# imdea-software/legosnark

Measured on AMD Instinct MI355X. Metric: alt_bn128 G1 MSM point-scalar pairs/s at n=2^20, higher is better.
Workload: dtype u32 limbs (254-bit Montgomery integers)

## Files before the change

### legosnark_amd/csrc/msm.hip

```cpp
#include <hip/hip_runtime.h>
#include <stdint.h>
#include <stdio.h>
#include <stdlib.h>
#include <string.h>
#include <algorithm>
#include <type_traits>
#include <vector>

#include "curves.h"
#include "fp29x2l.h"
#include "fs29.h"
#include "glv.h"
#include "msm.h"
#include "msm_plan.h"

namespace lsa {


template <class F, int K>
__global__ __launch_bounds__(256) void k_normalize(const Jac<F> *__restrict__ in, Aff<F> *__restrict__ out, size_t n) {
    size_t t = (size_t)blockIdx.x * blockDim.x + threadIdx.x;
    size_t base = t * K;
    if (base >= n) return;
    F prod[K];
// ... 447 lines not shown
            uint32_t gex = gi - gv, lex = li - lv;
            for (unsigned w = 0; w < wv; w++) { gex += wtot[0][w]; lex += wtot[1][w]; }
            lstart[threadIdx.x] = lex;
            lcur[threadIdx.x] = lex;
            gdst[threadIdx.x] = gex + tile_base[(size_t)t * pitch + threadIdx.x];
            if (blockIdx.x == 0) offs_c[threadIdx.x] = gex;
            if (threadIdx.x == Bc - 1) lstart[Bc] = lex + lv;
        }
    }
    __syncthreads();
    const size_t lo = (size_t)t * PART_TILE;
    const uint32_t fine_bits = cm.sh_hi;
    const uint32_t tlow = t & ((1u << (16 - fine_bits)) - 1);
    for (uint32_t j = 0; j < PART_TILE / 1024; j++) {
        const uint32_t il = threadIdx.x + j * 1024;
        const size_t i = lo + il;
        if (i >= n) break;
        const uint32_t seg = segment_of(segs, (uint32_t)i);
        wide_digits(scalars[i], pl, seg * B, [&](unsigned k, int32_t sd) {
            if (sd != 0) {
                const uint32_t b = (uint32_t)(sd < 0 ? -sd : sd) - 1;
                const uint32_t pos = atomicAdd(&lcur[cm.bin(b)], 1u);
                stage[pos] = (tlow << (16 + fine_bits)) | (cm.fine(b) << 16) | (k << 12) | (sd < 0 ? 0x800u : 0u) | il;
            }
        });
    }
    __syncthreads();
    for (uint32_t sg = threadIdx.x >> 5; sg < Bc; sg += 32) {
        const uint32_t a = lstart[sg], e = lstart[sg + 1], g = gdst[sg];
        for (uint32_t x = a + (lane & 31); x < e; x += 32) recs[g + (x - a)] = stage[x];
    }
}

__global__ __launch_bounds__(1024) void k_fine_sort_part(const uint32_t *__restrict__ recs, const uint32_t *__restrict__ offs_c,
                                                         const uint32_t *__restrict__ hist_c, const uint32_t *__restrict__ tile_base,
                                                         uint32_t pitch, uint32_t T, CoarseMap cm, SegList segs, uint32_t win_stride, uint32_t stage_cap,
                                                         uint32_t *__restrict__ entries, uint32_t *__restrict__ hist, uint32_t *__restrict__ offs) {
    __builtin_amdgcn_s_setprio(3);
    extern __shared__ __attribute__((aligned(16))) uint32_t sm[];
    __shared__ uint32_t wsum[16];
    const uint32_t sg = blockIdx.x, lo = offs_c[sg], ns = hist_c[sg];
    const uint32_t fine_bits = cm.sh_hi, FM = 1u << fine_bits, fmask = FM - 1, tbits = 16 - fine_bits;
    const uint32_t F = 1u << cm.bits(sg), bucket0 = cm.first(sg);
    uint32_t *cnt = sm, *cur = sm + FM, *col = sm + 2 * FM, *stage = col + T + 1;
    const unsigned lane = threadIdx.x & 63, wv = threadIdx.x >> 6;
    for (uint32_t x = threadIdx.x; x < F; x += 1024) cnt[x] = 0;
    for (uint32_t x = threadIdx.x; x < T; x += 1024) col[x] = tile_base[(size_t)x * pitch + sg];
    if (threadIdx.x == 0) col[T] = ns;
    auto scan_counters = [&]() {
        const uint32_t per = (F + 1023) >> 10, f0 = threadIdx.x * per;
        uint32_t sum = 0;
        for (uint32_t q = 0; q < per; q++) if (f0 + q < F) sum += cnt[f0 + q];
        uint32_t incl = sum;
#pragma unroll
        for (int d = 1; d < 64; d <<= 1) {
            const uint32_t u = __shfl_up(incl, d, 64);
            if ((int)lane >= d) incl += u;
        }
        if (lane == 63) wsum[wv] = incl;
        __syncthreads();
        uint32_t run = incl - sum;
        for (unsigned w = 0; w < wv; w++) run += wsum[w];
        for (uint32_t q = 0; q < per; q++) {
            if (f0 + q >= F) break;
            const uint32_t c = cnt[f0 + q];
            cur[f0 + q] = run;
            hist[(size_t)bucket0 + f0 + q] = c;
            offs[(size_t)bucket0 + f0 + q] = lo + run;
            run += c;
        }
    };
    auto entry_of = [&](uint32_t r, uint32_t p2) {
        uint32_t a = 0, e = (T + (1u << tbits) - 1) >> tbits;
        while (e - a > 1) {
            const uint32_t m = (a + e) >> 1;
            if (col[m << tbits] <= p2) a = m; else e = m;
        }
        const uint32_t i = ((a << tbits) | (r >> (16 + fine_bits))) * PART_TILE + (r & 0x7ffu);
        const uint32_t local = i - segs.off[segment_of(segs, i)];
        return (local + ((r >> 12) & 15u) * win_stride) | ((r & 0x800u) << 20);
    };
    if (ns <= stage_cap) {
        constexpr uint32_t NR = PART_STAGE / 1024;
        uint32_t r[NR];
#pragma unroll
        for (uint32_t u = 0; u < NR; u++) { const uint32_t p2 = threadIdx.x + u * 1024; r[u] = p2 < ns ? recs[lo + p2] : 0u; }
        __syncthreads();
        uint16_t rk[NR];
#pragma unroll
        for (uint32_t u = 0; u < NR; u++) {
            rk[u] = 0;
            if (threadIdx.x + u * 1024 < ns) rk[u] = (uint16_t)atomicAdd(&cnt[(r[u] >> 16) & fmask], 1u);
        }
        __syncthreads();
        scan_counters();
        __syncthreads();
#pragma unroll
        for (uint32_t u = 0; u < NR; u++) {
            const uint32_t p2 = threadIdx.x + u * 1024;
            if (p2 < ns) stage[cur[(r[u] >> 16) & fmask] + rk[u]] = entry_of(r[u], p2);
        }
        __syncthreads();
        for (uint32_t x = threadIdx.x; x < ns; x += 1024) entries[lo + x] = stage[x];
        return;
    }
    __syncthreads();
    constexpr uint32_t UNR = 8;
    for (uint32_t p0 = threadIdx.x; p0 < ns; p0 += 1024 * UNR) {
        uint32_t r[UNR];
#pragma unroll
        for (uint32_t u = 0; u < UNR; u++) { const uint32_t p2 = p0 + u * 1024; r[u] = p2 < ns ? recs[lo + p2] : 0u; }
#pragma unroll
        for (uint32_t u = 0; u < UNR; u++) if (p0 + u * 1024 < ns) (void)lds_inc_rank(cnt, (r[u] >> 16) & fmask);
    }
    __syncthreads();
    scan_counters();
    __syncthreads();
    for (uint32_t p0 = threadIdx.x; p0 < ns; p0 += 1024 * UNR) {
        uint32_t r[UNR];
#pragma unroll
        for (uint32_t u = 0; u < UNR; u++) { const uint32_t p2 = p0 + u * 1024; r[u] = p2 < ns ? recs[lo + p2] : 0u; }
#pragma unroll
        for (uint32_t u = 0; u < UNR; u++) {
            const uint32_t p2 = p0 + u * 1024;
            if (p2 >= ns) break;
            entries[lo + lds_inc_rank(cur, (r[u] >> 16) & fmask)] = entry_of(r[u], p2);
        }
    }
}

template <class Rec>
struct RecOps;
template <>
struct RecOps<uint64_t> {
    static constexpr uint32_t NF = 128;
    static __device__ __forceinline__ uint32_t fine(uint64_t r) { return (uint32_t)(r >> 32); }
    static __device__ __forceinline__ uint32_t entry(uint64_t r) { return (uint32_t)r; }
};
template <>
struct RecOps<uint32_t> {
    static constexpr uint32_t NF = 64;
    static __device__ __forceinline__ uint32_t fine(uint32_t r) { return (r >> 25) & 63u; }
    static __device__ __forceinline__ uint32_t entry(uint32_t r) { return r & 0x81ffffffu; }
};
template <class Rec>
__global__ __launch_bounds__(1024) void k_fine_sort(const Rec *__restrict__ recs, const uint32_t *__restrict__ offs_c,
                                                    const uint32_t *__restrict__ hist_c, uint32_t *__restrict__ entries,
                                                    uint32_t *__restrict__ hist, uint32_t *__restrict__ offs) {
    using O = RecOps<Rec>;
    constexpr uint32_t NF = O::NF;
// ... 1 lines not shown
    const uint32_t bin = blockIdx.x, lo = offs_c[bin], n = hist_c[bin];
    if (threadIdx.x < NF) cnt[threadIdx.x] = 0;
    __syncthreads();
    for (uint32_t j = threadIdx.x; j < n; j += 1024) atomicAdd(&cnt[O::fine(recs[lo + j])], 1u);
    __syncthreads();
    if (threadIdx.x < 64) {
        constexpr uint32_t PER = NF / 64;
        uint32_t c[PER], tot = 0;
#pragma unroll
        for (uint32_t q = 0; q < PER; q++) { c[q] = cnt[PER * threadIdx.x + q]; tot += c[q]; }
        uint32_t incl = tot;
#pragma unroll
        for (int d = 1; d < 64; d <<= 1) {
            uint32_t t = __shfl_up(incl, d, 64);
            if ((int)threadIdx.x >= d) incl += t;
        }
        uint32_t ex = incl - tot;
#pragma unroll
        for (uint32_t q = 0; q < PER; q++) {
            cur[PER * threadIdx.x + q] = ex;
            hist[(size_t)bin * NF + PER * threadIdx.x + q] = c[q];
            offs[(size_t)bin * NF + PER * threadIdx.x + q] = lo + ex;
            ex += c[q];
        }
    }
    __syncthreads();
    for (uint32_t j = threadIdx.x; j < n; j += 1024) {
        const Rec r = recs[lo + j];
        const uint32_t pos = atomicAdd(&cur[O::fine(r)], 1u);
        entries[lo + pos] = O::entry(r);
    }
}

__device__ __forceinline__ uint32_t size_bin(uint32_t cnt, uint32_t bin_shift) { return ((cnt - 1) >> bin_shift) + 1; }
template <class C>
__global__ __launch_bounds__(256) void k_size_hist(const uint32_t *__restrict__ hist, uint32_t nb, uint32_t thr, uint32_t *__restrict__ bin_count,
                                                   uint32_t group_size, uint32_t bin_shift) {
    bin_count += (group_size ? (blockIdx.x * 2048u) / group_size : 0u) * SIZE_BINS;
    __shared__ uint32_t lcnt[SIZE_BINS];
    for (uint32_t t = threadIdx.x; t < SIZE_BINS; t += 256) lcnt[t] = 0;
    __syncthreads();
    const uint32_t base = blockIdx.x * 2048 + threadIdx.x;
#pragma unroll
    for (int j = 0; j < 8; j++) {
        uint32_t g = base + j * 256;
        if (g < nb) { uint32_t cnt = hist[g]; if (cnt > 0 && cnt <= thr) atomicAdd(&lcnt[size_bin(cnt, bin_shift)], 1u); }
    }
    __syncthreads();
    for (uint32_t t = threadIdx.x; t < SIZE_BINS; t += 256) if (lcnt[t]) atomicAdd(&bin_count[t], lcnt[t]);
}
__global__ __launch_bounds__(256) void k_size_scan(const uint32_t *__restrict__ bin_count, uint32_t *__restrict__ bin_start, uint32_t ngroups) {
    __shared__ uint32_t lds[4];
    uint32_t carry = 0;
    for (uint32_t gidx = 0; gidx < ngroups; gidx++) {
        const uint32_t *bc = bin_count + gidx * SIZE_BINS;
        uint32_t *bs = bin_start + gidx * SIZE_BINS;
        uint32_t v[4], s = 0;
#pragma unroll
        for (int j = 0; j < 4; j++) {
            int bin = (int)SIZE_BINS - 1 - (int)(threadIdx.x * 4 + j);
            v[j] = (bin >= 1) ? bc[bin] : 0;
            s += v[j];
        }
        uint32_t tot;
        uint32_t run = carry + block_exclusive_scan_256(s, lds, &tot);
#pragma unroll
        for (int j = 0; j < 4; j++) {
            int bin = (int)SIZE_BINS - 1 - (int)(threadIdx.x * 4 + j);
            if (bin >= 1) bs[bin] = run;
            run += v[j];
        }
        carry += tot;
    }
    if (threadIdx.x == 0) bin_start[0] = carry;
}
template <class C>
__global__ __launch_bounds__(256) void k_size_scatter(const uint32_t *__restrict__ hist, uint32_t nb, uint32_t thr, const uint32_t *__restrict__ bin_start,
                                                      uint32_t *__restrict__ bin_cursor, uint32_t *__restrict__ perm,
                                                      uint32_t *__restrict__ heavy_list, uint32_t *__restrict__ heavy_count,
                                                      typename C::Acc *__restrict__ buckets, uint32_t group_size, uint32_t bin_shift,
                                                      uint32_t split) {
    const uint32_t goff = (group_size ? (blockIdx.x * 2048u) / group_size : 0u) * SIZE_BINS;
    bin_start += goff;
    bin_cursor += goff;
    __shared__ uint32_t lcnt[SIZE_BINS];
    for (uint32_t t = threadIdx.x; t < SIZE_BINS; t += 256) lcnt[t] = 0;
    __syncthreads();
    const uint32_t base = blockIdx.x * 2048 + threadIdx.x;
    uint32_t cnt[8], rank[8];
#pragma unroll
    for (int j = 0; j < 8; j++) {
        uint32_t g = base + j * 256;
        cnt[j] = 0; rank[j] = 0;
        if (g < nb) {
            cnt[j] = hist[g];
            if (cnt[j] == 0) { for (uint32_t h = 0; h < split; h++) buckets[(size_t)g * split + h] = C::inf(); }
            else if (cnt[j] > thr) heavy_list[atomicAdd(heavy_count, 1u)] = g;
            else rank[j] = atomicAdd(&lcnt[size_bin(cnt[j], bin_shift)], 1u);
        }
    }
    __syncthreads();
    for (uint32_t t = threadIdx.x; t < SIZE_BINS; t += 256) {
        uint32_t c = lcnt[t];
        lcnt[t] = c ? atomicAdd(&bin_cursor[t], c) : 0;
    }
    __syncthreads();
#pragma unroll
    for (int j = 0; j < 8; j++) {
        uint32_t g = base + j * 256;
        if (g < nb && cnt[j] > 0 && cnt[j] <= thr) {
            const uint32_t bin = size_bin(cnt[j], bin_shift);
            perm[bin_start[bin] + lcnt[bin] + rank[j]] = g;
        }
    }
}

typedef uint32_t u32x4 __attribute__((ext_vector_type(4)));
template <class B> struct RawBase {
    static_assert(sizeof(B) % 16 == 0, "packed bases are whole 16-byte vectors");
    u32x4 q[sizeof(B) / 16];
};
template <class B>
__device__ __forceinline__ RawBase<B> load_base16(const B *__restrict__ p) {
    const u32x4 *src = reinterpret_cast<const u32x4 *>(p);
    RawBase<B> r;
#pragma unroll
    for (int i = 0; i < (int)(sizeof(B) / 16); i++) r.q[i] = src[i];
    return r;
}
template <class B>
__device__ __forceinline__ B packed_base(RawBase<B> r) {
    B b;
    uint32_t *dst = reinterpret_cast<uint32_t *>(&b);
#pragma unroll
    for (int i = 0; i < (int)(sizeof(B) / 16); i++) {
        asm("" : "+v"(r.q[i]));
        dst[4 * i] = r.q[i].x; dst[4 * i + 1] = r.q[i].y; dst[4 * i + 2] = r.q[i].z; dst[4 * i + 3] = r.q[i].w;
    }
    return b;
}
template <class C> struct RotatedLoads { static constexpr bool value = true; };
template <> struct RotatedLoads<CurveG2> { static constexpr bool value = false; };
template <class C, uint32_t ACC_SPLIT, bool ROTATED = RotatedLoads<C>::value>
__device__ __forceinline__ void accumulate_body(const typename C::Base *__restrict__ bases, const uint32_t *__restrict__ entries,
                                                const uint32_t *__restrict__ offs, const uint32_t *__restrict__ hist,
                                                const uint32_t *__restrict__ perm, const uint32_t *__restrict__ nperm,
// ... 103 lines not shown
    o[4 + part] = acc.ZZ.v;
    o[6 + part] = acc.ZZZ.v;
}

template <class A>
__device__ __forceinline__ A shfl_down_acc(const A &p, unsigned delta) {
    A r;
    constexpr int NW = sizeof(A) / 4;
    const uint32_t *src = reinterpret_cast<const uint32_t *>(&p);
    uint32_t *dst = reinterpret_cast<uint32_t *>(&r);
#pragma unroll
    for (int i = 0; i < NW; i++) dst[i] = __shfl_down(src[i], delta, 64);
    return r;
}

enum TailKernel { TAIL_HEAVY, TAIL_REDUCE1_LANE, TAIL_REDUCE2_LANE };
template <class C, TailKernel K> struct PairedAdd { static constexpr bool value = false; };
template <> struct PairedAdd<CurveG1, TAIL_HEAVY> { static constexpr bool value = true; };
template <> struct PairedAdd<CurveG1, TAIL_REDUCE1_LANE> { static constexpr bool value = true; };

template <class C, bool PAIRED = false>
__device__ __forceinline__ typename C::Acc wave_sum(typename C::Acc v, unsigned lane) {
    for (unsigned d = 32; d >= 1; d >>= 1) {
        typename C::Acc t = shfl_down_acc(v, d);
        if (lane + d < 64) v = C::template add<PAIRED>(v, t);
    }
    return v;
}

__global__ __launch_bounds__(256) void k_heavy_plan(const uint32_t *__restrict__ hist, const uint32_t *__restrict__ heavy_list,
                                                    const uint32_t *__restrict__ heavy_count, uint32_t *__restrict__ chunk_off) {
    __shared__ uint32_t lds[4];
    __shared__ uint32_t s_chunk;
    const uint32_t nh = *heavy_count;
    uint32_t carry = 0;
    for (uint32_t base = 0; base < nh; base += 256) {
        uint32_t h = base + threadIdx.x;
        uint32_t tot;
        (void)block_exclusive_scan_256(h < nh ? hist[heavy_list[h]] : 0, lds, &tot);
        carry += tot;
    }
    if (threadIdx.x == 0) {
        uint32_t chunk = HEAVY_CHUNK;
        while (chunk < 4096u && carry / (2 * chunk) >= 2048u) chunk *= 2;
        s_chunk = chunk;
    }
    __syncthreads();
    const uint32_t chunk = s_chunk;
    carry = 0;
    for (uint32_t base = 0; base < nh; base += 256) {
        uint32_t h = base + threadIdx.x;
        uint32_t v = h < nh ? (hist[heavy_list[h]] + chunk - 1) / chunk : 0;
        uint32_t tot;
        uint32_t ex = block_exclusive_scan_256(v, lds, &tot);
        if (h < nh) chunk_off[h] = carry + ex;
        carry += tot;
    }
    if (threadIdx.x == 0) { chunk_off[nh] = carry; chunk_off[nh + 1] = chunk; }
}

template <class C>
__global__ __launch_bounds__(64) void k_accumulate_heavy(const typename C::Base *__restrict__ bases, const uint32_t *__restrict__ entries,
                                                         const uint32_t *__restrict__ offs, const uint32_t *__restrict__ hist,
                                                         const uint32_t *__restrict__ heavy_list, const uint32_t *__restrict__ heavy_count,
                                                         const uint32_t *__restrict__ chunk_off, typename C::Acc *__restrict__ partials) {
    const uint32_t nh = *heavy_count;
    if (nh == 0) return;
    const uint32_t total = chunk_off[nh], chunk = chunk_off[nh + 1];
    const unsigned lane = threadIdx.x;
    for (uint32_t v = blockIdx.x; v < total; v += gridDim.x) {
        uint32_t lo = 0, hi = nh;
        while (hi - lo > 1) { uint32_t mid = (lo + hi) >> 1; if (chunk_off[mid] <= v) lo = mid; else hi = mid; }
        const uint32_t g = heavy_list[lo];
        const uint32_t cnt = hist[g];
        const uint32_t start = (v - chunk_off[lo]) * chunk;
        const uint32_t end = start + chunk < cnt ? start + chunk : cnt;
        const uint32_t *e = entries + offs[g];
        typename C::Acc acc = C::inf();
        uint32_t j = start + lane;
        if constexpr (!RotatedLoads<C>::value) {
            for (; j < end; j += 64) {
                uint32_t w = e[j];
                acc = C::madd(acc, bases[w & 0x3fffffffu], (w >> 31) != 0, ((w >> 30) & 1) != 0);
            }
        } else if (j < end) {
            const uint32_t last = j + (end - 1 - j) / 64 * 64;
            auto word = [&](uint32_t k) { return e[k < last ? k : last]; };
            uint32_t w = word(j), wn = word(j + 64);
            RawBase<typename C::Base> cur = load_base16(bases + (w & 0x3fffffffu));
            for (; j < end; j += 64) {
                const uint32_t wnn = word(j + 128);
// ... 539 lines not shown
    Aff<F> *tmp = (Aff<F> *)g_prep_ws.ptr;
    hipLaunchKernelGGL((k_normalize<F, K>), dim3(blocks), dim3(256), 0, st, d_in, tmp, n);
    hipLaunchKernelGGL((k_convert_bases<C>), dim3((unsigned)((n + 255) / 256)), dim3(256), 0, st, tmp, (typename C::Base *)d_out, n);
    HIPCHK(hipGetLastError());
    return LSA_OK;
}
template int prepare_bases<Fq>(const Jac<Fq> *, void *, size_t, hipStream_t);
template int prepare_bases<Fq2>(const Jac<Fq2> *, void *, size_t, hipStream_t);

template <class F>
int normalize_to_affine(const Jac<F> *d_in, Aff<F> *d_out, size_t n, hipStream_t st) {
    if (n == 0) return LSA_OK;
    constexpr int K = 8;
    size_t threads = (n + K - 1) / K;
    unsigned blocks = (unsigned)((threads + 255) / 256);
    hipLaunchKernelGGL((k_normalize<F, K>), dim3(blocks), dim3(256), 0, st, d_in, d_out, n);
    HIPCHK(hipGetLastError());
    return LSA_OK;
}
template int normalize_to_affine<Fq>(const Jac<Fq> *, Aff<Fq> *, size_t, hipStream_t);
template int normalize_to_affine<Fq2>(const Jac<Fq2> *, Aff<Fq2> *, size_t, hipStream_t);

static MsmSwitches &switches() {
    static MsmSwitches sw = [] {
        const auto is_one = [](const char *name) { const char *e = getenv(name); return e && e[0] == '1'; };
        MsmSwitches v;
        v.no_rec32 = getenv("LSA_NO_REC32") != nullptr;
        v.no_part = getenv("LSA_NO_PART") != nullptr;
        if (const char *e = getenv("LSA_WIDE_SPLIT")) v.wide_split = (uint32_t)atoi(e);
        v.g2_pair = is_one("LSA_G2_PAIR");
        v.no_reduce_bits = getenv("LSA_NO_REDUCE_BITS") != nullptr;
        v.no_lane_l1 = getenv("LSA_NO_LANE_L1") != nullptr;
        v.g2_lane_l1 = is_one("LSA_G2_LANE_L1");
        if (const char *e = getenv("LSA_WIDE_BIG_MIN")) v.wide_big_min = (size_t)atoll(e);
        return v;
    }();
    return sw;
}
unsigned msm_table_windows(int , size_t n) { return table_copies(n); }

static size_t g_merge_min = 0;
static bool g_merge_min_explicit = false;
void msm_set_merge_min(size_t n) {
    g_merge_min = n;
    g_merge_min_explicit = n != 0;
    switches().table_use_min = n ? n : 1;
}
size_t msm_merge_min() {
    if (g_merge_min == 0) {
        const char *e = getenv("LSA_PRECOMPUTE_MIN");
        g_merge_min = e && atoll(e) > 0 ? (size_t)atoll(e) : (size_t)1 << 19;
    }
    return g_merge_min;
}
bool msm_merge_min_is_explicit() { return g_merge_min_explicit; }
bool msm_uses_table(size_t n) { return n >= switches().table_use_min; }

template <class C>
__global__ __launch_bounds__(256) void k_shift_window(const typename C::Base *__restrict__ prev, Jac<typename C::Field> *__restrict__ out,
                                                      size_t n, unsigned c) {
    size_t i = (size_t)blockIdx.x * blockDim.x + threadIdx.x;
    if (i >= n) return;
    typename C::Acc p = C::madd(C::inf(), prev[i], false, false);
    for (unsigned j = 0; j < c; j++) p = C::dbl(p);
    out[i] = C::to_jac(p);
}
// ... 65 lines not shown
        entries = (uint32_t *)(ws + p.front[F_ENTRIES]);
        heavy_list = (uint32_t *)(ws + p.front[F_HEAVY]);
        chunk_off = (uint32_t *)(ws + p.front[F_CHOFF]);
        hpart = (A *)(ws + p.front[F_HPART]);
        recs = ws + p.front[F_RECS];
        hist_c = p.fine ? (uint32_t *)(ws + p.front[F_CHIST]) : hist;
        offs_c = p.fine ? (uint32_t *)(ws + p.front[F_COFFS]) : offs;
        buckets = (A *)(tws + p.tail[T_BUCKETS]);
        wave_out = (A *)(tws + p.tail[T_WAVE]);
        window_sums = (A *)(tws + p.tail[T_WIN]);
        res = tws + p.tail[T_RES];
    }
};

struct Marks {
    hipEvent_t *ev;
    void operator()(int i, hipStream_t s) const { if (ev) (void)hipEventRecord(ev[i], s); }
};

template <class C>
static void launch_sort(const PipelinePlan &p, const MsmBuffers<typename C::Acc> &b, const Fr *d_scalars, const SegList &segs, hipStream_t st,
                        const Marks &mark) {
    const size_t n = p.n;
    if (p.wide) {
        hipLaunchKernelGGL(k_hist_wide, dim3(p.wtiles), dim3(1024), p.lds_hist_wide, st, d_scalars, n, segs, p.pl, p.B, p.Bc, p.cm, p.pitch, p.wtile, b.tile_hist);
        mark(1, st);
        hipLaunchKernelGGL(k_tile_scan_rows, dim3((p.Bc + 31) / 32), dim3(1024), 0, st, b.tile_hist, p.Bc, p.wtiles, p.pitch, b.tile_base, b.hist_c, b.heavy_count,
                           b.bin_count, (uint32_t)(3 * SIZE_BINS));
        mark(2, st);
        if (p.part) {
            hipLaunchKernelGGL(k_partition, dim3(p.wtiles), dim3(1024), p.lds_partition, st, d_scalars, n, segs, p.pl, p.B, p.Bc, p.cm, p.pitch,
                               b.tile_hist, b.hist_c, b.offs_c, b.tile_base, (uint32_t *)b.recs);
            hipLaunchKernelGGL(k_fine_sort_part, dim3(p.Bc), dim3(1024), p.lds_fine_sort_part, st, (const uint32_t *)b.recs, b.offs_c, b.hist_c,
                               b.tile_base, p.pitch, p.wtiles, p.cm, segs, p.win_stride, p.stage_cap, b.entries, b.hist, b.offs);
        } else if (p.rec32) {
            hipLaunchKernelGGL(k_scatter_wide<2>, dim3(p.wtiles), dim3(1024), p.lds_scatter_wide, st, d_scalars, n, segs, p.pl, p.B, p.Bc, p.pitch, p.wtile, b.hist_c, b.offs_c, b.tile_base, b.recs, p.win_stride);
            hipLaunchKernelGGL(k_fine_sort<uint32_t>, dim3(p.Bc), dim3(1024), 0, st, (const uint32_t *)b.recs, b.offs_c, b.hist_c, b.entries, b.hist, b.offs);
        } else if (p.fine) {
            hipLaunchKernelGGL(k_scatter_wide<1>, dim3(p.wtiles), dim3(1024), p.lds_scatter_wide, st, d_scalars, n, segs, p.pl, p.B, p.Bc, p.pitch, p.wtile, b.hist_c, b.offs_c, b.tile_base, b.recs, p.win_stride);
            hipLaunchKernelGGL(k_fine_sort<uint64_t>, dim3(p.Bc), dim3(1024), 0, st, (const uint64_t *)b.recs, b.offs_c, b.hist_c, b.entries, b.hist, b.offs);
        } else {
            hipLaunchKernelGGL(k_scatter_wide<0>, dim3(p.wtiles), dim3(1024), p.lds_scatter_wide, st, d_scalars, n, segs, p.pl, p.B, p.Bc, p.pitch, p.wtile, b.hist_c, b.offs_c, b.tile_base, (void *)b.entries, p.win_stride);
        }
        mark(3, st);
    } else {
        hipLaunchKernelGGL((k_digits<C::GLV>), dim3((unsigned)((n + 255) / 256)), dim3(256), 0, st, d_scalars, n, p.c, p.nwin, b.digits);
        hipLaunchKernelGGL(k_rank, dim3(p.ntiles, p.nwin), dim3(1024), p.lds_rank, st, b.digits, p.nv, p.B, p.ntiles, b.rank, b.tile_hist, 0u);
        hipLaunchKernelGGL(k_tile_scan, dim3((p.nb + 255) / 256), dim3(256), 0, st, b.tile_hist, p.B, p.ntiles, p.nb, b.tile_base, b.hist);
        mark(1, st);
        hipLaunchKernelGGL(k_scan_sums, dim3(p.scan_blocks), dim3(256), 0, st, b.hist, p.nb, b.bsum);
        hipLaunchKernelGGL(k_scan_blocks, dim3(1), dim3(256), 0, st, b.bsum, p.scan_blocks);
        hipLaunchKernelGGL(k_scan_final, dim3(p.scan_blocks), dim3(256), 0, st, b.hist, b.bsum, p.nb, b.offs);
        mark(2, st);
        hipLaunchKernelGGL(k_scatter, dim3(p.ntiles, p.nwin), dim3(1024), p.lds_scatter, st, b.digits, b.rank, b.offs, b.tile_base, p.nv, n, p.B, p.ntiles, b.entries, 0u);
        mark(3, st);
    }
}

template <class C>
static int launch_accumulate(const PipelinePlan &p, const MsmBuffers<typename C::Acc> &b, const typename C::Base *d_bases, hipStream_t st, const Marks &mark) {
    constexpr bool g2 = std::is_same<C, CurveG2>::value;
    if (!p.wide || p.reuse_sort) {
        HIPCHK(hipMemsetAsync(b.heavy_count, 0, 4, st));
        HIPCHK(hipMemsetAsync(b.bin_count, 0, (size_t)3 * SIZE_BINS * 4, st));
    }
    const unsigned sb = (p.nb + 2047) / 2048;
    const uint32_t gsz = 0u, ngroups = 1;
    hipLaunchKernelGGL((k_size_hist<C>), dim3(sb), dim3(256), 0, st, b.hist, p.nb, p.heavy_threshold, b.bin_count, gsz, p.bin_shift);
    hipLaunchKernelGGL(k_size_scan, dim3(1), dim3(256), 0, st, b.bin_count, b.bin_start, ngroups);
    hipLaunchKernelGGL((k_size_scatter<C>), dim3(sb), dim3(256), 0, st, b.hist, p.nb, p.heavy_threshold, b.bin_start, b.bin_cursor, b.perm, b.heavy_list, b.heavy_count, b.buckets, gsz, p.bin_shift, p.split);
    mark(4, st);
    const dim3 one_lane((p.nb + 255) / 256), two_lanes((p.nb * 2 + 255) / 256);
    if (g2 && p.g2_pair) {
        if constexpr (g2) hipLaunchKernelGGL(k_accumulate_g2_pair, two_lanes, dim3(256), 0, st, d_bases, b.entries, b.offs, b.hist, b.perm, b.bin_start, b.buckets);
    } else if (g2 && p.split == 1) {
        if constexpr (g2) hipLaunchKernelGGL(k_accumulate_g2_occ2, one_lane, dim3(256), 0, st, d_bases, b.entries, b.offs, b.hist, b.perm, b.bin_start, b.buckets);
    } else if (p.split == 1) {
        hipLaunchKernelGGL((k_accumulate<C, 1u>), one_lane, dim3(256), 0, st, d_bases, b.entries, b.offs, b.hist, b.perm, b.bin_start, b.buckets);
    } else {
        hipLaunchKernelGGL((k_accumulate<C, 2u>), two_lanes, dim3(256), 0, st, d_bases, b.entries, b.offs, b.hist, b.perm, b.bin_start, b.buckets);
    }
    hipLaunchKernelGGL(k_heavy_plan, dim3(1), dim3(256), 0, st, b.hist, b.heavy_list, b.heavy_count, b.chunk_off);
    hipLaunchKernelGGL((k_accumulate_heavy<C>), dim3(4096), dim3(64), 0, st, d_bases, b.entries, b.offs, b.hist,
                       b.heavy_list, b.heavy_count, b.chunk_off, b.hpart);
    hipLaunchKernelGGL((k_heavy_finish<C>), dim3(256), dim3(64), 0, st, b.heavy_list, b.heavy_count, b.chunk_off, b.hpart, b.buckets, p.split);
    mark(5, st);
    return LSA_OK;
}

template <class C>
static int launch_tail(const PipelinePlan &p, const MsmBuffers<typename C::Acc> &b, Jac<typename C::Field> *d_out, hipStream_t tail, bool inline_tail,
                       bool lane_l1, TailBuf &tb, TailBuf &prev, const Marks &mark) {
    using A = typename C::Acc;
    using J = Jac<typename C::Field>;
    constexpr bool g1 = std::is_same<C, CurveG1>::value;
    if (p.big)
        hipLaunchKernelGGL((k_reduce1_lane<C>), dim3(p.kw * ((p.T + 63) / 64)), dim3(64), 0, tail, b.buckets, p.B, p.L, p.split, b.wave_out);
    else
        hipLaunchKernelGGL((k_reduce1<C>), dim3(p.kw * p.wpw), dim3(64), 0, tail, b.buckets, p.B, p.L, p.logL, p.wpw, p.split, b.wave_out);
    A *lvl_in = b.wave_out, *lvl_out = b.window_sums;
    uint32_t m = p.wpw, lm = p.big ? p.logL : p.logL + 4;
    J *res = inline_tail ? d_out : (J *)b.res;
    const auto level = [&](bool lane) {
        const uint32_t m_out = (m + 15) / 16;
        if (lane) hipLaunchKernelGGL((k_reduce2_lane<C>), dim3((m_out + 63) / 64), dim3(64), 0, tail, lvl_in, m, m_out, lm, lvl_out);
        else hipLaunchKernelGGL((k_reduce2<C>), dim3(p.kw * m_out), dim3(64), 0, tail, lvl_in, m, m_out, lm, lvl_out);
        std::swap(lvl_in, lvl_out);
        m = m_out;
        lm += 4;
    };
    level(lane_l1);
    if (p.bits_tail) {
        uint32_t nbits = 0;
        while ((1u << nbits) < m) nbits++;
        const uint32_t G = (m + 511) / 512;
// ... 151 lines not shown
```

### legosnark_amd/csrc/msm_plan.h

```cpp
#pragma once
#include <stdint.h>
#include <stddef.h>
#include "bn254_constants.h"
#include "fp.h"

namespace lsa {

struct WidePlan {
    unsigned nwin;
    unsigned c;
    unsigned copy_step;
    unsigned start[32];
    unsigned width[32];
};

struct TableGrid {
    unsigned ncopies;
    unsigned pos[33];
};
inline TableGrid table_grid(size_t n_table) {
    TableGrid t;
    const unsigned nbig = n_table >= ((size_t)6 << 20) ? 12u : 13u;
    const unsigned base = 255 / nbig, rem = 255 % nbig;
    unsigned bit = 0;
// ... 45 lines not shown
struct CoarseMap {
    uint32_t half, sh_lo, sh_hi, nlo;
    LSA_HD uint32_t bin(uint32_t b) const { return b < half ? b >> sh_lo : nlo + ((b - half) >> sh_hi); }
    LSA_HD uint32_t fine(uint32_t b) const { return b < half ? b & ((1u << sh_lo) - 1) : (b - half) & ((1u << sh_hi) - 1); }
    LSA_HD uint32_t first(uint32_t bin_) const { return bin_ < nlo ? bin_ << sh_lo : half + ((bin_ - nlo) << sh_hi); }
    LSA_HD uint32_t bits(uint32_t bin_) const { return bin_ < nlo ? sh_lo : sh_hi; }
};

inline unsigned msm_window_bits(size_t n) {
    unsigned lg = 0;
    while ((size_t(1) << (lg + 1)) <= n) lg++;
    int c = (int)lg - 4;
    if (c < 8) c = 8;
    if (c > 16) c = 16;
    return (unsigned)c;
}

inline unsigned num_windows(unsigned c) { return (255 + c - 1) / c; }

inline uint32_t wide_tile(uint32_t nwin, size_t n) {
    if (n <= 4096) return 256u;
    if (n <= 16384) return 1024u;
    return nwin > 15 ? 2048u : 4096u;
}

struct MsmSwitches {
    bool no_rec32 = false;
    bool no_part = false;
    uint32_t wide_split = 1;
    bool g2_pair = false;
    bool no_reduce_bits = false;
    bool no_lane_l1 = false;
    bool g2_lane_l1 = false;
    size_t wide_big_min = (size_t)1 << 16;
    size_t table_use_min = 1;
};

struct MsmShape {
    int group;
    size_t acc_bytes;
    size_t jac_bytes;
    bool glv;
    size_t n;
    uint32_t nseg;
    size_t table_stride;
    bool blocking, reuse_sort;
};

enum PlanStatus {
    PLAN_OK = 0,
    PLAN_N_TOO_LARGE,
    PLAN_SEGMENTS_NEED_COPIES,
    PLAN_TABLE_TOO_LARGE,
    PLAN_BIN_SPACE,
};

inline size_t align_up(size_t x, size_t a) { return (x + a - 1) / a * a; }

struct WsRegion { size_t off, bytes; };
enum FrontRegion {
    F_HIST,
    F_OFFS,
    F_BSUM,
    F_BINS,
    F_PERM,
    F_DIGITS,
// ... 8 lines not shown
    F_CHIST,
    F_COFFS,
    F_REGIONS
};
enum TailRegion {
    T_BUCKETS,
    T_WAVE,
    T_WIN,
    T_RES,
    T_REGIONS
};
template <int N>
struct WsLayout {
    WsRegion r[N];
    size_t total;
    size_t operator[](int i) const { return r[i].off; }
    void carve(int i, size_t bytes) {
        r[i].off = i == 0 ? 0 : total;
        r[i].bytes = bytes;
        total = align_up(r[i].off + bytes, 256);
    }
};

struct PipelinePlan {
    PlanStatus status;
    size_t n;
    uint32_t nseg;
    bool reuse_sort;
    bool wide;
    bool glv;
    bool fine;
    bool rec32;
    bool part;
    bool big;
    WidePlan pl;
    unsigned c, nwin;
    size_t nv, ne;
    uint32_t B, nb;
    uint32_t Bc;
    CoarseMap cm;
    uint32_t fine_bits;
    uint32_t win_stride;
    uint32_t ntiles, wtile, wtiles;
    size_t rows;
    uint32_t pitch;
    uint32_t nscan, scan_blocks;
    uint32_t split;
    bool g2_pair;
    uint32_t heavy_threshold, bin_shift, max_heavy;
    size_t max_chunks;
    uint32_t L, logL, T, wpw, kw;
    bool bits_tail;
    bool lane_l1_shape;
    size_t lds_hist_wide, lds_scatter_wide, lds_rank, lds_scatter, lds_partition, lds_fine_sort_part;
    uint32_t fixed_words, stage_cap;
    WsLayout<F_REGIONS> front;
    WsLayout<T_REGIONS> tail;
};

inline unsigned table_copies(size_t n_table) { return table_grid(n_table).ncopies; }
inline WidePlan wide_plan(size_t n_table, size_t n_call, unsigned nseg, const MsmSwitches &sw) {
    return wide_plan_for(n_table, nseg == 1 && n_call >= sw.wide_big_min);
}

inline PipelinePlan plan_pipeline(const MsmShape &sh, const MsmSwitches &sw) {
    PipelinePlan p = {};
// ... 31 lines not shown
    }
    const size_t ne = nv * nwin;
    const bool big = wide && B > 4096;
    const uint32_t split = wide ? (sw.wide_split == 2 ? 2u : 1u) : 2u;
    const uint32_t L = big ? (B / 65536 > 1 ? B / 65536 : 1) : (B > 4096 ? B / 4096 : 1);
    uint32_t logL = 0;
    while ((1u << logL) < L) logL++;
    const uint32_t T = B / L;
    const uint32_t wpw = big ? T : (T + 15) / 16;
    const uint32_t kw = wide ? nseg : nwin;
    const uint32_t avg_pop = (uint32_t)(ne / nb + 1);
    uint32_t pop_lo = avg_pop;
    if (wide && big) {
        unsigned nfull = 0;
        for (unsigned k = 0; k < nwin; k++) nfull += pl.width[k] == c;
        pop_lo = (uint32_t)(((uint64_t)n * (nfull + 2 * (nwin - nfull))) / B + 1);
    }
    const uint32_t pop = wide ? pop_lo : avg_pop;
    const uint32_t heavy_threshold = (wide && !big) ? 4u : (2 * pop + 32 > 64 ? 2 * pop + 32 : 64u);
    uint32_t bin_shift = 0;
    while (((heavy_threshold - 1) >> bin_shift) + 1 > SIZE_BINS - 1) bin_shift++;
    const uint32_t max_heavy = (uint32_t)(ne / heavy_threshold + 1 < nb ? ne / heavy_threshold + 1 : nb);
    const size_t max_chunks = ne / HEAVY_CHUNK + max_heavy + 1;
    const uint32_t nscan = wide ? Bc : nb;
    const uint32_t scan_blocks = (nscan + SCAN_PER_BLOCK - 1) / SCAN_PER_BLOCK;
    const uint32_t ntiles = (uint32_t)((nv + SORT_TILE - 1) / SORT_TILE);
    const uint32_t wtile = part ? PART_TILE : wide_tile(nwin, n);
    const uint32_t wtiles = (uint32_t)((n + wtile - 1) / wtile);
    const size_t rows = wide ? wtiles : (size_t)nwin * ntiles;
    const uint32_t pitch = wide ? Bc + 96 : Bc;

    p.status = PLAN_OK;
    p.wide = wide; p.glv = glv; p.fine = fine; p.rec32 = rec32; p.part = part; p.big = big;
    p.pl = pl; p.c = c; p.nwin = nwin; p.nv = nv; p.ne = ne; p.B = B; p.nb = nb; p.Bc = Bc; p.cm = cm; p.fine_bits = fine_bits;
    p.win_stride = wide ? (uint32_t)(table_stride * pl.copy_step) : 0u;
    p.ntiles = ntiles; p.wtile = wtile; p.wtiles = wtiles; p.rows = rows; p.pitch = pitch; p.nscan = nscan; p.scan_blocks = scan_blocks;
    p.split = split; p.g2_pair = sh.group == 2 && split == 1 && sw.g2_pair; p.heavy_threshold = heavy_threshold; p.bin_shift = bin_shift; p.max_heavy = max_heavy; p.max_chunks = max_chunks;
    p.L = L; p.logL = logL; p.T = T; p.wpw = wpw; p.kw = kw;
    p.bits_tail = !sw.no_reduce_bits && sh.blocking && big && kw == 1 && nseg == 1 && wpw >= 4096 && (wpw / 16) <= 8192;
    p.lane_l1_shape = !sw.no_lane_l1 && (sh.group == 1 || sw.g2_lane_l1) && !sh.blocking && !sh.reuse_sort && big && kw == 1 && nseg == 1 && wpw >= 16384;

    p.lds_hist_wide = (size_t)((Bc + 1) / 2) * 4;
    p.lds_scatter_wide = (size_t)Bc * 4;
    p.lds_rank = (size_t)B * 2;
    p.lds_scatter = (size_t)B * 4;
    p.lds_partition = (size_t)nwin * PART_TILE * 4;
    if (part) {
        p.fixed_words = 2 * (1u << cm.sh_hi) + wtiles + 1;
        p.stage_cap = p.fixed_words + PART_STAGE <= LDS_MAX_FINE_SORT_PART / 4 ? PART_STAGE : 0u;
    }
    p.lds_fine_sort_part = (size_t)(p.fixed_words + p.stage_cap) * 4;

    p.front.carve(F_HIST, (size_t)nb * 4 + 256);
    p.front.carve(F_OFFS, (size_t)nb * 4);
    p.front.carve(F_BSUM, (size_t)scan_blocks * 4);
    p.front.carve(F_BINS, (size_t)3 * SIZE_BINS * 4);
    p.front.carve(F_PERM, (size_t)nb * 4);
    p.front.carve(F_DIGITS, wide ? 0 : ne * 4);
    p.front.carve(F_RANK, wide ? 0 : ne * 2);
    p.front.carve(F_THIST, rows * pitch * 2);
    p.front.carve(F_TBASE, rows * pitch * 4);
    p.front.carve(F_ENTRIES, ne * 4);
    p.front.carve(F_HEAVY, (size_t)max_heavy * 4);
    p.front.carve(F_CHOFF, (size_t)(max_heavy + 2) * 4);
    p.front.carve(F_HPART, max_chunks * sh.acc_bytes);
    p.front.carve(F_RECS, fine ? ne * (part || rec32 ? 4 : 8) : 0);
// ... 59 lines not shown
```

Baseline: 837.4 million.

## Fuse bucket size histogram into fine sort and heavy planning into size scatter

```diff
diff --git a/legosnark_amd/csrc/msm.hip b/legosnark_amd/csrc/msm.hip
--- a/legosnark_amd/csrc/msm.hip
+++ b/legosnark_amd/csrc/msm.hip
@@ -503,13 +503,19 @@
     }
 }
 
+__device__ __forceinline__ uint32_t size_bin(uint32_t cnt, uint32_t bin_shift) { return ((cnt - 1) >> bin_shift) + 1; }
+
 __global__ __launch_bounds__(1024) void k_fine_sort_part(const uint32_t *__restrict__ recs, const uint32_t *__restrict__ offs_c,
                                                          const uint32_t *__restrict__ hist_c, const uint32_t *__restrict__ tile_base,
                                                          uint32_t pitch, uint32_t T, CoarseMap cm, SegList segs, uint32_t win_stride, uint32_t stage_cap,
-                                                         uint32_t *__restrict__ entries, uint32_t *__restrict__ hist, uint32_t *__restrict__ offs) {
+                                                         uint32_t *__restrict__ entries, uint32_t *__restrict__ hist, uint32_t *__restrict__ offs,
+                                                         uint32_t thr, uint32_t bin_shift, uint32_t *__restrict__ bin_count) {
     __builtin_amdgcn_s_setprio(3);
     extern __shared__ __attribute__((aligned(16))) uint32_t sm[];
     __shared__ uint32_t wsum[16];
+    __shared__ uint32_t lbin[SIZE_BINS];
+    const uint32_t nbins = thr ? min(size_bin(thr, bin_shift) + 1, (uint32_t)SIZE_BINS) : 0u;
+    for (uint32_t x = threadIdx.x; x < nbins; x += 1024) lbin[x] = 0;
     const uint32_t sg = blockIdx.x, lo = offs_c[sg], ns = hist_c[sg];
     const uint32_t fine_bits = cm.sh_hi, FM = 1u << fine_bits, fmask = FM - 1, tbits = 16 - fine_bits;
     const uint32_t F = 1u << cm.bits(sg), bucket0 = cm.first(sg);
@@ -539,7 +545,11 @@
             hist[(size_t)bucket0 + f0 + q] = c;
             offs[(size_t)bucket0 + f0 + q] = lo + run;
             run += c;
-        }
+            if (c > 0 && c <= thr) atomicAdd(&lbin[size_bin(c, bin_shift)], 1u);
+        }
+    };
+    auto flush_bins = [&]() {
+        for (uint32_t x = threadIdx.x; x < nbins; x += 1024) { const uint32_t v = lbin[x]; if (v) atomicAdd(&bin_count[x], v); }
     };
     auto entry_of = [&](uint32_t r, uint32_t p2) {
         uint32_t a = 0, e = (T + (1u << tbits) - 1) >> tbits;
@@ -566,6 +576,7 @@
         __syncthreads();
         scan_counters();
         __syncthreads();
+        flush_bins();
 #pragma unroll
         for (uint32_t u = 0; u < NR; u++) {
             const uint32_t p2 = threadIdx.x + u * 1024;
@@ -587,6 +598,7 @@
     __syncthreads();
     scan_counters();
     __syncthreads();
+    flush_bins();
     for (uint32_t p0 = threadIdx.x; p0 < ns; p0 += 1024 * UNR) {
         uint32_t r[UNR];
 #pragma unroll
@@ -654,7 +666,6 @@
     }
 }
 
-__device__ __forceinline__ uint32_t size_bin(uint32_t cnt, uint32_t bin_shift) { return ((cnt - 1) >> bin_shift) + 1; }
 template <class C>
 __global__ __launch_bounds__(256) void k_size_hist(const uint32_t *__restrict__ hist, uint32_t nb, uint32_t thr, uint32_t *__restrict__ bin_count,
                                                    uint32_t group_size, uint32_t bin_shift) {
@@ -696,17 +707,66 @@
     }
     if (threadIdx.x == 0) bin_start[0] = carry;
 }
-template <class C>
+__device__ __forceinline__ void heavy_plan_body(const uint32_t *__restrict__ hist, const uint32_t *__restrict__ heavy_list, const uint32_t nh,
+                                                uint32_t *__restrict__ chunk_off, uint32_t *lds, uint32_t *s_chunk) {
+    uint32_t carry = 0;
+    for (uint32_t base = 0; base < nh; base += 256) {
+        uint32_t h = base + threadIdx.x;
+        uint32_t tot;
+        (void)block_exclusive_scan_256(h < nh ? hist[heavy_list[h]] : 0, lds, &tot);
+        carry += tot;
+    }
+    if (threadIdx.x == 0) {
+        uint32_t chunk = HEAVY_CHUNK;
+        while (chunk < 4096u && carry / (2 * chunk) >= 2048u) chunk *= 2;
+        *s_chunk = chunk;
+    }
+    __syncthreads();
+    const uint32_t chunk = *s_chunk;
+    carry = 0;
+    for (uint32_t base = 0; base < nh; base += 256) {
+        uint32_t h = base + threadIdx.x;
+        uint32_t v = h < nh ? (hist[heavy_list[h]] + chunk - 1) / chunk : 0;
+        uint32_t tot;
+        uint32_t ex = block_exclusive_scan_256(v, lds, &tot);
+        if (h < nh) chunk_off[h] = carry + ex;
+        carry += tot;
+    }
+    if (threadIdx.x == 0) { chunk_off[nh] = carry; chunk_off[nh + 1] = chunk; }
+}
+
+template <class C, bool FUSED = false>
 __global__ __launch_bounds__(256) void k_size_scatter(const uint32_t *__restrict__ hist, uint32_t nb, uint32_t thr, const uint32_t *__restrict__ bin_start,
                                                       uint32_t *__restrict__ bin_cursor, uint32_t *__restrict__ perm,
                                                       uint32_t *__restrict__ heavy_list, uint32_t *__restrict__ heavy_count,
                                                       typename C::Acc *__restrict__ buckets, uint32_t group_size, uint32_t bin_shift,
-                                                      uint32_t split) {
+                                                      uint32_t split, const uint32_t *__restrict__ bin_count = nullptr, uint32_t *__restrict__ nperm = nullptr,
+                                                      uint32_t *__restrict__ ticket = nullptr, uint32_t *__restrict__ chunk_off = nullptr) {
     const uint32_t goff = (group_size ? (blockIdx.x * 2048u) / group_size : 0u) * SIZE_BINS;
     bin_start += goff;
     bin_cursor += goff;
     __shared__ uint32_t lcnt[SIZE_BINS];
+    __shared__ uint32_t lstart[FUSED ? SIZE_BINS : 1];
+    __shared__ uint32_t lds[4];
     for (uint32_t t = threadIdx.x; t < SIZE_BINS; t += 256) lcnt[t] = 0;
+    if constexpr (FUSED) {
+        uint32_t v[4], s = 0;
+#pragma unroll
+        for (int j = 0; j < 4; j++) {
+            const int bin = (int)SIZE_BINS - 1 - (int)(threadIdx.x * 4 + j);
+            v[j] = (bin >= 1) ? bin_count[bin] : 0;
+            s += v[j];
+        }
+        uint32_t tot;
+        uint32_t run = block_exclusive_scan_256(s, lds, &tot);
+#pragma unroll
+        for (int j = 0; j < 4; j++) {
+            const int bin = (int)SIZE_BINS - 1 - (int)(threadIdx.x * 4 + j);
+            if (bin >= 1) lstart[bin] = run;
+            run += v[j];
+        }
+        if (blockIdx.x == 0 && threadIdx.x == 0) *nperm = tot;
+    }
     __syncthreads();
     const uint32_t base = blockIdx.x * 2048 + threadIdx.x;
     uint32_t cnt[8], rank[8];
@@ -717,7 +777,11 @@
         if (g < nb) {
             cnt[j] = hist[g];
             if (cnt[j] == 0) { for (uint32_t h = 0; h < split; h++) buckets[(size_t)g * split + h] = C::inf(); }
-            else if (cnt[j] > thr) heavy_list[atomicAdd(heavy_count, 1u)] = g;
+            else if (cnt[j] > thr) {
+                const uint32_t h = atomicAdd(heavy_count, 1u);
+                if constexpr (FUSED) __hip_atomic_store(&heavy_list[h], g, __ATOMIC_RELAXED, __HIP_MEMORY_SCOPE_AGENT);
+                else heavy_list[h] = g;
+            }
             else rank[j] = atomicAdd(&lcnt[size_bin(cnt[j], bin_shift)], 1u);
         }
     }
@@ -732,8 +796,26 @@
         uint32_t g = base + j * 256;
         if (g < nb && cnt[j] > 0 && cnt[j] <= thr) {
             const uint32_t bin = size_bin(cnt[j], bin_shift);
-            perm[bin_start[bin] + lcnt[bin] + rank[j]] = g;
-        }
+            perm[(FUSED ? lstart[bin] : bin_start[bin]) + lcnt[bin] + rank[j]] = g;
+        }
+    }
+    if constexpr (FUSED) {
+        __shared__ uint32_t s_last, s_chunk;
+        asm volatile("s_waitcnt vmcnt(0)" ::: "memory");
+        __syncthreads();
+        if (threadIdx.x == 0) {
+            const uint32_t drawn = __hip_atomic_fetch_add(ticket, 1u, __ATOMIC_RELAXED, __HIP_MEMORY_SCOPE_AGENT);
+            const bool last = drawn == gridDim.x - 1;
+            if (last) {
+                __builtin_amdgcn_fence(__ATOMIC_ACQUIRE, "agent");
+                asm volatile("s_waitcnt vmcnt(0)" ::: "memory");
+            }
+            s_last = last;
+        }
+        __syncthreads();
+        if (!s_last) return;
+        const uint32_t nh = __hip_atomic_load(heavy_count, __ATOMIC_RELAXED, __HIP_MEMORY_SCOPE_AGENT);
+        heavy_plan_body(hist, heavy_list, nh, chunk_off, lds, &s_chunk);
     }
 }
 
@@ -903,31 +985,7 @@
                                                     const uint32_t *__restrict__ heavy_count, uint32_t *__restrict__ chunk_off) {
     __shared__ uint32_t lds[4];
     __shared__ uint32_t s_chunk;
-    const uint32_t nh = *heavy_count;
-    uint32_t carry = 0;
-    for (uint32_t base = 0; base < nh; base += 256) {
-        uint32_t h = base + threadIdx.x;
-        uint32_t tot;
-        (void)block_exclusive_scan_256(h < nh ? hist[heavy_list[h]] : 0, lds, &tot);
-        carry += tot;
-    }
-    if (threadIdx.x == 0) {
-        uint32_t chunk = HEAVY_CHUNK;
-        while (chunk < 4096u && carry / (2 * chunk) >= 2048u) chunk *= 2;
-        s_chunk = chunk;
-    }
-    __syncthreads();
-    const uint32_t chunk = s_chunk;
-    carry = 0;
-    for (uint32_t base = 0; base < nh; base += 256) {
-        uint32_t h = base + threadIdx.x;
-        uint32_t v = h < nh ? (hist[heavy_list[h]] + chunk - 1) / chunk : 0;
-        uint32_t tot;
-        uint32_t ex = block_exclusive_scan_256(v, lds, &tot);
-        if (h < nh) chunk_off[h] = carry + ex;
-        carry += tot;
-    }
-    if (threadIdx.x == 0) { chunk_off[nh] = carry; chunk_off[nh + 1] = chunk; }
+    heavy_plan_body(hist, heavy_list, *heavy_count, chunk_off, lds, &s_chunk);
 }
 
 template <class C>
@@ -1533,6 +1591,7 @@
         v.no_reduce_bits = getenv("LSA_NO_REDUCE_BITS") != nullptr;
         v.no_lane_l1 = getenv("LSA_NO_LANE_L1") != nullptr;
         v.g2_lane_l1 = is_one("LSA_G2_LANE_L1");
+        v.no_fused_order = is_one("LSA_NO_FUSED_ORDER");
         if (const char *e = getenv("LSA_WIDE_BIG_MIN")) v.wide_big_min = (size_t)atoll(e);
         return v;
     }();
@@ -1664,7 +1723,8 @@
             hipLaunchKernelGGL(k_partition, dim3(p.wtiles), dim3(1024), p.lds_partition, st, d_scalars, n, segs, p.pl, p.B, p.Bc, p.cm, p.pitch,
                                b.tile_hist, b.hist_c, b.offs_c, b.tile_base, (uint32_t *)b.recs);
             hipLaunchKernelGGL(k_fine_sort_part, dim3(p.Bc), dim3(1024), p.lds_fine_sort_part, st, (const uint32_t *)b.recs, b.offs_c, b.hist_c,
-                               b.tile_base, p.pitch, p.wtiles, p.cm, segs, p.win_stride, p.stage_cap, b.entries, b.hist, b.offs);
+                               b.tile_base, p.pitch, p.wtiles, p.cm, segs, p.win_stride, p.stage_cap, b.entries, b.hist, b.offs,
+                               p.fused_order ? p.heavy_threshold : 0u, p.bin_shift, b.bin_count);
         } else if (p.rec32) {
             hipLaunchKernelGGL(k_scatter_wide<2>, dim3(p.wtiles), dim3(1024), p.lds_scatter_wide, st, d_scalars, n, segs, p.pl, p.B, p.Bc, p.pitch, p.wtile, b.hist_c, b.offs_c, b.tile_base, b.recs, p.win_stride);
             hipLaunchKernelGGL(k_fine_sort<uint32_t>, dim3(p.Bc), dim3(1024), 0, st, (const uint32_t *)b.recs, b.offs_c, b.hist_c, b.entries, b.hist, b.offs);
@@ -1698,9 +1758,15 @@
     }
     const unsigned sb = (p.nb + 2047) / 2048;
     const uint32_t gsz = 0u, ngroups = 1;
-    hipLaunchKernelGGL((k_size_hist<C>), dim3(sb), dim3(256), 0, st, b.hist, p.nb, p.heavy_threshold, b.bin_count, gsz, p.bin_shift);
-    hipLaunchKernelGGL(k_size_scan, dim3(1), dim3(256), 0, st, b.bin_count, b.bin_start, ngroups);
-    hipLaunchKernelGGL((k_size_scatter<C>), dim3(sb), dim3(256), 0, st, b.hist, p.nb, p.heavy_threshold, b.bin_start, b.bin_cursor, b.perm, b.heavy_list, b.heavy_count, b.buckets, gsz, p.bin_shift, p.split);
+    if (p.fused_order) {
+        hipLaunchKernelGGL((k_size_scatter<C, true>), dim3(sb), dim3(256), 0, st, b.hist, p.nb, p.heavy_threshold, b.bin_start, b.bin_cursor, b.perm, b.heavy_list, b.heavy_count, b.buckets, gsz, p.bin_shift, p.split,
+                           b.bin_count, b.bin_start, b.bin_cursor, b.chunk_off);
+    } else {
+        hipLaunchKernelGGL((k_size_hist<C>), dim3(sb), dim3(256), 0, st, b.hist, p.nb, p.heavy_threshold, b.bin_count, gsz, p.bin_shift);
+        hipLaunchKernelGGL(k_size_scan, dim3(1), dim3(256), 0, st, b.bin_count, b.bin_start, ngroups);
+        hipLaunchKernelGGL((k_size_scatter<C>), dim3(sb), dim3(256), 0, st, b.hist, p.nb, p.heavy_threshold, b.bin_start, b.bin_cursor, b.perm, b.heavy_list, b.heavy_count, b.buckets, gsz, p.bin_shift, p.split,
+                           (const uint32_t *)nullptr, (uint32_t *)nullptr, (uint32_t *)nullptr, (uint32_t *)nullptr);
+    }
     mark(4, st);
     const dim3 one_lane((p.nb + 255) / 256), two_lanes((p.nb * 2 + 255) / 256);
     if (g2 && p.g2_pair) {
@@ -1712,7 +1778,7 @@
     } else {
         hipLaunchKernelGGL((k_accumulate<C, 2u>), two_lanes, dim3(256), 0, st, d_bases, b.entries, b.offs, b.hist, b.perm, b.bin_start, b.buckets);
     }
-    hipLaunchKernelGGL(k_heavy_plan, dim3(1), dim3(256), 0, st, b.hist, b.heavy_list, b.heavy_count, b.chunk_off);
+    if (!p.fused_order) hipLaunchKernelGGL(k_heavy_plan, dim3(1), dim3(256), 0, st, b.hist, b.heavy_list, b.heavy_count, b.chunk_off);
     hipLaunchKernelGGL((k_accumulate_heavy<C>), dim3(4096), dim3(64), 0, st, d_bases, b.entries, b.offs, b.hist,
                        b.heavy_list, b.heavy_count, b.chunk_off, b.hpart);
     hipLaunchKernelGGL((k_heavy_finish<C>), dim3(256), dim3(64), 0, st, b.heavy_list, b.heavy_count, b.chunk_off, b.hpart, b.buckets, p.split);
diff --git a/legosnark_amd/csrc/msm_plan.h b/legosnark_amd/csrc/msm_plan.h
--- a/legosnark_amd/csrc/msm_plan.h
+++ b/legosnark_amd/csrc/msm_plan.h
@@ -101,6 +101,7 @@
     bool no_reduce_bits = false;
     bool no_lane_l1 = false;
     bool g2_lane_l1 = false;
+    bool no_fused_order = false;
     size_t wide_big_min = (size_t)1 << 16;
     size_t table_use_min = 1;
 };
@@ -175,6 +176,7 @@
     bool fine;
     bool rec32;
     bool part;
+    bool fused_order;
     bool big;
     WidePlan pl;
     unsigned c, nwin;
@@ -272,6 +274,7 @@
 
     p.status = PLAN_OK;
     p.wide = wide; p.glv = glv; p.fine = fine; p.rec32 = rec32; p.part = part; p.big = big;
+    p.fused_order = part && !sh.reuse_sort && !sw.no_fused_order;
     p.pl = pl; p.c = c; p.nwin = nwin; p.nv = nv; p.ne = ne; p.B = B; p.nb = nb; p.Bc = Bc; p.cm = cm; p.fine_bits = fine_bits;
     p.win_stride = wide ? (uint32_t)(table_stride * pl.copy_step) : 0u;
     p.ntiles = ntiles; p.wtile = wtile; p.wtiles = wtiles; p.rows = rows; p.pitch = pitch; p.nscan = nscan; p.scan_blocks = scan_blocks;
```

New measurement: 834.9 million. No clear change (-0.3%).
